# TheJacksonLaboratory/cnn_autoencoder

Measured on NVIDIA B200. Metric: wsi_encode_decode_megapixels_per_sec, higher is better.
Workload: dtype f16

## Files before the change

### cnn_autoencoder_b200/csrc/igemm_conv.cu

```cuda
#include <stdlib.h>
#include <string.h>

#include "cae_common.cuh"
#include "eb_device.cuh"

namespace {

constexpr int kMaxTaps = 9;
constexpr int kMaxSA = 6;
constexpr int kMaxSB = 12;
constexpr int kMaxEpiWarps = 12;
constexpr int kThreads = 128 + 32 * kMaxEpiWarps;

enum { EPI_ACT = 0, EPI_LATENT = 1, EPI_IMAGE = 2, EPI_PROJ = 3 };

constexpr int kProjN = 32;
constexpr int kProjK = 128;
constexpr int kProjStageBytes = (kProjK / 8) * 256 * 16;
constexpr int kProjWBytes = (kProjK / 8) * kProjN * 16;
__host__ __device__ inline int proj_slot(int kh, int kw) {
  const int slot[3][3] = {{12, 24, 27}, {16, 0, 3}, {19, 6, 9}};
  return slot[kh][kw];
}

struct IgTap {
  uint32_t a_off;
  uint32_t acc;
};

constexpr int kMaxItems = 18;
constexpr int kMaxStages = 9;

struct IgItem {
  uint32_t a_off16, b_off16, d_off, first;
};

struct IgParams {
  int n_img, dom_h, dom_w;
  int tiles_x, tiles_per_img, n_tiles;
  int mt, n_taps, n_chunks, ck;
  int N, n_acc, n_buf, tmem_cols;
  int PH, PW, n_par, par_stride;
  int a_stage_bytes, a_box_bytes, b_stage_bytes, sa, sb;
  int tpb, b_tap_bytes;
  int n_pass;
  int pass_tap0[2];
  int n_stages[2];
  IgItem items[2][2][kMaxItems];
  int item_start[2][2][kMaxStages + 1];
  int epi_warps;
  int debug;
  int org_y, org_x;
  uint32_t lbo_a, sbo_a, lbo_b, sbo_b, idesc;
  IgTap taps[kMaxTaps];
  const uint8_t *wpack;
  size_t wpack_half_bytes;
  int resident;
  uint32_t b_chunk16;
  int up;
  int c_out, pre_act, post_act;
  const float *bias;
  ActView out, skip;
  float *aux;
  int out_h, out_w;
  uint32_t out_pitch, out_ps, out_is, skip_pitch, skip_ps, skip_is;
  int pair_store;
  int quant;
  int q_smem;
  int q_core_min, q_core_len;
  cae_eb_tables qt;
  float *q_yq;
  int32_t *q_sym, *q_hist, *q_status;
  double *q_rate;
  ActView q_pl;
  uint32_t q_pitch, q_ps, q_is;
  const uint8_t *proj_w;
  __half *proj_out;
  uint32_t idesc2;
};

struct TapDef {
  int par, dy, dx, acc, kh, kw;
};

int build_taps(int kind, bool merged, TapDef *t) {
  int n = 0;
  if (kind == CAE_CONV_S1) {
    for (int kh = 0; kh < 3; ++kh)
      for (int kw = 0; kw < 3; ++kw) t[n++] = {0, kh, kw, 0, kh, kw};
  } else if (kind == CAE_CONV_S2) {
    for (int kh = 0; kh < 3; ++kh)
      for (int kw = 0; kw < 3; ++kw)
        t[n++] = {((kh & 1) << 1) | ((kw + CAE_COL_PAD) & 1), kh >> 1,
                  ((kw + CAE_COL_PAD) >> 1) - 1, 0, kh, kw};
  } else if (kind == CAE_CONVT_S1) {
    for (int dy = 0; dy < 3; ++dy)
      for (int dx = 0; dx < 3; ++dx) t[n++] = {0, dy, dx, 0, 2 - dy, 2 - dx};
  } else if (merged) {
    for (int dy = 0; dy < 2; ++dy)
      for (int dx = 0; dx < 2; ++dx) t[n++] = {0, dy, dx, 0, -1, -1};
  } else {
    for (int py = 0; py < 2; ++py)
      for (int px = 0; px < 2; ++px)
        for (int dy = 0; dy <= py; ++dy)
          for (int dx = 0; dx <= px; ++dx)
            t[n++] = {0, dy, dx, py * 2 + px, py + 1 - 2 * dy, px + 1 - 2 * dx};
  }
  return n;
}

inline int round_up(int a, int b) { return (a + b - 1) / b * b; }

inline bool is_merged(int kind, int c_out) { return kind == CAE_CONVT_S2 && 4 * c_out <= 16; }

inline int mma_n(int kind, int c_out) {
  return is_merged(kind, c_out) ? 16 : round_up(c_out, 16);
}

inline bool use_pair(int kind, int c_out) {
  return !is_merged(kind, c_out) && mma_n(kind, c_out) == 128 && cae_knob(CAE_KNOB_IGEMM_PAIR_MMA);
}

inline int auto_ck(int kind, int c_in_p, bool merged = false, bool pair = false) {
  if (pair && c_in_p % 32 == 0) {
    if (const char *e = cae_knob(CAE_KNOB_IGEMM_CK_PAIR)) {
      const int v = atoi(e);
      if ((v == 16 || v == 32 || v == 64) && c_in_p % v == 0) return v;
// ... 387 lines not shown
    return;
  }

#pragma unroll 1
  for (int part = 0; part < 2; ++part) {
    if (part == 1 && !second) break;
    float v[16];
#pragma unroll
    for (int i = 0; i < 16; ++i) v[i] = __uint_as_float(part ? r1[i] : r0[i]);
    const int c0 = part ? c_second : c_first;
    const int ox = ox0 + (p.up == 2 ? part : 0);
    if (p.bias) {
      if (c0 + 16 <= p.c_out) {
        const float4 *bp = reinterpret_cast<const float4 *>(p.bias + c0);
#pragma unroll
        for (int q = 0; q < 4; ++q) {
          const float4 bv = __ldg(bp + q);
          v[4 * q] += bv.x;
          v[4 * q + 1] += bv.y;
          v[4 * q + 2] += bv.z;
          v[4 * q + 3] += bv.w;
        }
      } else {
#pragma unroll
        for (int i = 0; i < 16; ++i)
          if (c0 + i < p.c_out) v[i] += __ldg(p.bias + c0 + i);
      }
    }
    if (pre_s != 1.f) {
#pragma unroll
      for (int i = 0; i < 16; ++i) v[i] = fmaxf(v[i], v[i] * pre_s);
    }
    if (p.skip.ptr) {
      const uint32_t off = pixel_unit(p.skip.fmt, p.skip_pitch, p.skip_ps, p.skip_is,
                                      p.skip.planes, n, oy + 1, ox + 1) +
                           (uint32_t)(c0 >> 3) * p.skip_ps;
      const uint4 *sp = reinterpret_cast<const uint4 *>(p.skip.ptr) + off;
#pragma unroll
      for (int h = 0; h < 2; ++h) {
        const uint4 sv = __ldg(sp + h * p.skip_ps);
        const __half2 *sh = reinterpret_cast<const __half2 *>(&sv);
#pragma unroll
        for (int k = 0; k < 4; ++k) {
          const float2 f = __half22float2(sh[k]);
          v[h * 8 + 2 * k] += f.x;
          v[h * 8 + 2 * k + 1] += f.y;
        }
      }
    }
    if (post_s != 1.f) {
#pragma unroll
      for (int i = 0; i < 16; ++i) v[i] = fmaxf(v[i], v[i] * post_s);
    }
    if (EPI == EPI_LATENT) {
      if (valid) {
        float *o = reinterpret_cast<float *>(p.out.ptr) +
                   (((size_t)n * p.c_out + c0) * p.out_h + oy) * p.out_w + ox;
        const size_t cs = (size_t)p.out_h * p.out_w;
#pragma unroll
        for (int i = 0; i < 16; ++i)
          if (c0 + i < p.c_out) o[i * cs] = v[i];
      }
      if (fused_q) quant_emit16(p, qs, v, c0, n, oy, ox, valid, q_bits);
    } else {
      const uint4 lo = pack8(v), hi = pack8(v + 8);
      const uint32_t off = pixel_unit(p.out.fmt, p.out_pitch, p.out_ps, p.out_is, p.out.planes,
                                      n, oy + 1, ox + 1) + (uint32_t)(c0 >> 3) * p.out_ps;
      uint4 *dst = reinterpret_cast<uint4 *>(p.out.ptr) + off;
      dst[0] = lo;
      dst[p.out_ps] = hi;
      if (p.out.halo == CAE_HALO_REFLECT &&
          (oy == 1 || oy == p.out.H - 2 || ox == 1 || ox == p.out.W - 2))
        store_halo2(p, n, c0 >> 3, oy, ox, lo, hi);
    }
  }
}

template <int EPI, int FAST, int PAIR>
__global__ void __launch_bounds__(EPI == EPI_PROJ ? 128 + 32 * 17 : (FAST == 1 ? 128 + 32 * 16 : kThreads), 1)
igemm_conv_kernel(const __grid_constant__ CUtensorMap tmA, const __grid_constant__ IgParams p) {
  extern __shared__ uint8_t smem_raw[];
  __shared__ __align__(8) uint64_t a_full[kMaxSA], a_empty[kMaxSA];
  __shared__ __align__(8) uint64_t b_full[kMaxSB], b_empty[kMaxSB];
  __shared__ __align__(8) uint64_t acc_full[2], acc_empty[2];
  __shared__ __align__(8) uint64_t b_peer[kMaxSB];
  __shared__ __align__(8) uint64_t u_full, u_free, d2_full;
  __shared__ uint32_t tmem_base_s;

  const int warp = threadIdx.x >> 5, lane = threadIdx.x & 31;
  const uint32_t rank = PAIR ? cluster_ctarank() : 0u;
  const int unit0 = PAIR ? (int)(blockIdx.x >> 1) : (int)blockIdx.x;
  const int unit_step = PAIR ? (int)(gridDim.x >> 1) : (int)gridDim.x;
  const int n_units = (PAIR ? (p.n_tiles + 1) >> 1 : p.n_tiles) * p.n_pass;
  const uint32_t smem_base = (smem_u32(smem_raw) + 1023u) & ~1023u;
  uint8_t *smem = smem_raw + (smem_base - smem_u32(smem_raw));
  uint8_t *smem_a = smem;
  uint8_t *smem_b = smem + (size_t)p.sa * p.a_stage_bytes;
  QuantSmem qs{nullptr, nullptr, nullptr};
  if (EPI == EPI_LATENT && p.quant && p.q_smem) {
    float *q0 = reinterpret_cast<float *>(smem_b + (size_t)p.sb * p.b_stage_bytes);
    const int nl = p.c_out * p.q_core_len, nh = p.q_hist ? nl : 0;
    for (int i = threadIdx.x; i < p.c_out; i += blockDim.x) q0[i] = p.qt.medians[i];
    for (int i = threadIdx.x; i < nl; i += blockDim.x) {
      const int c = i / p.q_core_len, k = i - c * p.q_core_len;
      q0[p.c_out + i] = p.qt.lut[(size_t)c * p.qt.lut_len + (p.q_core_min - p.qt.lut_min) + k];
    }
    int *h0 = reinterpret_cast<int *>(q0 + p.c_out + nl);
    for (int i = threadIdx.x; i < nh; i += blockDim.x) h0[i] = 0;
    qs.med = q0;
    qs.lut = q0 + p.c_out;
    qs.hist = nh ? h0 : nullptr;
  }

  if (threadIdx.x == 0) {
    for (int i = 0; i < p.sa; ++i) {
      mbar_init(&a_full[i], 1);
      mbar_init(&a_empty[i], 2);
    }
    for (int i = 0; i < p.sb; ++i) {
      mbar_init(&b_full[i], 1);
      mbar_init(&b_empty[i], 2);
    }
    for (int i = 0; i < 2; ++i) {
      mbar_init(&acc_full[i], 2);
      mbar_init(&acc_empty[i], (uint32_t)p.epi_warps * (PAIR ? 2u : 1u));
    }
    if (PAIR) {
      for (int i = 0; i < p.sb; ++i) mbar_init(&b_peer[i], 1);
    }
    if (EPI == EPI_PROJ) {
      mbar_init(&u_full, (uint32_t)p.epi_warps * (PAIR ? 2u : 1u));
      mbar_init(&u_free, 1);
      mbar_init(&d2_full, 1);
    }
    fence_barrier_init();
  }
  uint8_t *u_stage = smem_b + (size_t)p.sb * p.b_stage_bytes;
  uint8_t *proj_w_s = u_stage + kProjStageBytes;
  if (EPI == EPI_PROJ) {
    const uint4 *src = reinterpret_cast<const uint4 *>(
        p.proj_w + (PAIR ? kProjWBytes + rank * (kProjWBytes / 2) : 0));
    uint4 *dst = reinterpret_cast<uint4 *>(proj_w_s);
    for (int i = threadIdx.x; i < kProjWBytes / 16 / (PAIR ? 2 : 1); i += blockDim.x)
      dst[i] = __ldg(src + i);
    fence_proxy_async();
  }
  if (warp == 3) tmem_alloc_g<PAIR>(&tmem_base_s, (uint32_t)p.tmem_cols);
  if (warp == 0 && lane == 0) prefetch_tensormap(&tmA);
  tc_fence_before();
  if (PAIR) cluster_sync_all(); else __syncthreads();
  tc_fence_after();
  const uint32_t tmem_base = tmem_base_s;

  if (warp == 0) {
    if (lane == 0) {
      uint32_t it = 0;
      for (int vt = unit0; vt < n_units; vt += unit_step) {
        const int tile = PAIR ? (vt / p.n_pass) * 2 + (int)rank : vt / p.n_pass;
        const int n = tile / p.tiles_per_img, rem = tile - n * p.tiles_per_img;
        const int ty = rem / p.tiles_x, tx = rem - ty * p.tiles_x;
        const int y0 = ty * 16 + p.org_y, x0 = tx * 8 * p.mt + p.org_x;
        for (int ch = 0; ch < p.n_chunks; ++ch, ++it) {
          const int s = it % p.sa;
          mbar_wait(&a_empty[s], ((it / p.sa) & 1) ^ 1);
          if (PAIR) {
            if (rank == 0) mbar_expect_tx(&a_full[s], 2u * (uint32_t)(p.n_par * p.a_box_bytes));
            const uint32_t bar = mapa_u32(smem_u32(&a_full[s]), 0);
            for (int par = 0; par < p.n_par; ++par)
              tma_load_4d_pair(&tmA, bar,
                               smem_a + (size_t)s * p.a_stage_bytes + (size_t)par * p.par_stride,
                               x0 * 8, y0, ch * (p.ck >> 3), n * p.n_par + par);
            continue;
          }
          if (p.debug & 1) { mbar_arrive(&a_full[s]); continue; }
          mbar_expect_tx(&a_full[s], (uint32_t)(p.n_par * p.a_box_bytes));
          for (int par = 0; par < p.n_par; ++par)
            tma_load_4d(&tmA, &a_full[s],
                        smem_a + (size_t)s * p.a_stage_bytes + (size_t)par * p.par_stride, x0 * 8,
                        y0, ch * (p.ck >> 3), n * p.n_par + par);
        }
      }
    }
  } else if (warp == 1) {
    if (lane == 0) {
      uint32_t it = 0;
      const uint8_t *wsrc = p.wpack + (size_t)rank * p.wpack_half_bytes;
      if (p.resident) {
        mbar_expect_tx(&b_full[0], (uint32_t)p.b_stage_bytes);
        for (int k = 0; k < p.n_chunks * p.n_taps; ++k)
          bulk_load_1d(smem_b + (size_t)k * p.b_tap_bytes, wsrc + (size_t)k * p.b_tap_bytes,
                       (uint32_t)p.b_tap_bytes, &b_full[0]);
      }
      for (int vt = unit0; vt < n_units && !p.resident; vt += unit_step) {
        const int pass = vt % p.n_pass;
        for (int ch = 0; ch < p.n_chunks; ++ch) {
          for (int st = 0; st < p.n_stages[pass]; ++st, ++it) {
            const int s = it % p.sb;
            mbar_wait(&b_empty[s], ((it / p.sb) & 1) ^ 1);
            if (p.debug & 2) { mbar_arrive(&b_full[s]); continue; }
            mbar_expect_tx(&b_full[s], (uint32_t)p.b_stage_bytes);
            bulk_load_1d(smem_b + (size_t)s * p.b_stage_bytes,
                         wsrc + (size_t)(ch * p.n_taps + p.pass_tap0[pass] + st * p.tpb) *
                                    p.b_tap_bytes,
                         (uint32_t)p.b_stage_bytes, &b_full[s]);
          }
        }
      }
    }
  }
  if (PAIR && rank != 0 && (warp == 2 || warp == 3)) {
    if (warp == 3 && lane == 0) {
      if (p.resident) {
        mbar_wait(&b_full[0], 0);
        mbar_arrive_cluster(mapa_u32(smem_u32(&b_peer[0]), 0));
      }
      uint32_t it = 0;
      for (int vt = unit0; vt < n_units && !p.resident; vt += unit_step) {
        const int pass = vt % p.n_pass;
        for (int k = 0; k < p.n_chunks * p.n_stages[pass]; ++k, ++it) {
          const int s = it % p.sb;
          mbar_wait(&b_full[s], (it / p.sb) & 1);
          mbar_arrive_cluster(mapa_u32(smem_u32(&b_peer[s]), 0));
        }
      }
    }
  } else if (warp == 2 || warp == 3) {
    const int issuer = warp - 2;
    const bool leader = elect_one();
    const uint32_t a_hi = ((p.sbo_a >> 4) & 0x3FFFu) | (1u << 14);
    const uint32_t b_hi = ((p.sbo_b >> 4) & 0x3FFFu) | (1u << 14);
    const uint32_t a_lbo = ((p.lbo_a >> 4) & 0x3FFFu) << 16;
    const uint32_t b_lbo = ((p.lbo_b >> 4) & 0x3FFFu) << 16;
    const uint32_t a_kstep = (2 * p.lbo_a) >> 4, b_kstep = (2 * p.lbo_b) >> 4;
    const uint32_t sa_base = smem_base >> 4;
    const uint32_t sb_base = (smem_base + (uint32_t)(p.sa * p.a_stage_bytes)) >> 4;
    const uint32_t a_stage16 = (uint32_t)p.a_stage_bytes >> 4;
    const uint32_t b_stage16 = (uint32_t)p.b_stage_bytes >> 4;
    const uint32_t idesc = p.idesc;
    const int ksteps = p.ck >> 4;
    const uint32_t buf_cols = (uint32_t)(p.mt * p.n_acc * p.N);
    const bool no_mma = (p.debug & 4) != 0;
    uint32_t j = 0;
    int sA = 0, sB = 0;
    uint32_t phA = 0, phB = 0;
    const bool resident = p.resident != 0;
    if (resident) {
      mbar_wait(&b_full[0], 0);
      if (PAIR) mbar_wait_cluster(&b_peer[0], 0);
    }
    for (int vt = unit0; vt < n_units; vt += unit_step, ++j) {
      const int pass = vt % p.n_pass;
      const int n_stages = p.n_stages[pass];
      const int buf = j % p.n_buf;
      if (PAIR) mbar_wait_cluster(&acc_empty[buf], ((j / p.n_buf) & 1) ^ 1);
      else mbar_wait(&acc_empty[buf], ((j / p.n_buf) & 1) ^ 1);
      tc_fence_after();
      const uint32_t d_buf = tmem_base + (uint32_t)buf * buf_cols;
      for (int ch = 0; ch < p.n_chunks; ++ch) {
        if (PAIR) mbar_wait_cluster(&a_full[sA], phA); else mbar_wait(&a_full[sA], phA);
        const uint32_t a_stage = ((sa_base + (uint32_t)sA * a_stage16) & 0x3FFFu) | a_lbo;
        const uint32_t later = ch > 0 ? 1u : 0u;
        for (int st = 0; st < n_stages; ++st) {
          if (!resident) {
            mbar_wait(&b_full[sB], phB);
            if (PAIR) mbar_wait_cluster(&b_peer[sB], phB);
          }
          tc_fence_after();
          const uint32_t b_stage =
              ((sb_base + (resident ? (uint32_t)ch * p.b_chunk16 : (uint32_t)sB * b_stage16)) & 0x3FFFu) | b_lbo;
          const int i1 = p.item_start[pass][issuer][st + 1];
          for (int i = p.item_start[pass][issuer][st]; i < i1; ++i) {
            const IgItem it = p.items[pass][issuer][i];
            const uint32_t d = d_buf + it.d_off;
            uint32_t a_lo = a_stage + it.a_off16, b_lo = b_stage + it.b_off16;
            uint32_t flag = later | (it.first ^ 1u);
            if (leader && !no_mma) {
#pragma unroll 4
              for (int k = 0; k < ksteps; ++k) {
                umma_f16_lohi_g<PAIR>(d, a_lo, a_hi, b_lo, b_hi, idesc, flag);
                a_lo += a_kstep;
                b_lo += b_kstep;
                flag = 1u;
              }
            }
          }
          if (leader) {
            if (!resident) umma_commit_g<PAIR>(&b_empty[sB]);
            if (st == n_stages - 1) umma_commit_g<PAIR>(&a_empty[sA]);
            if (st == n_stages - 1 && ch == p.n_chunks - 1) umma_commit_g<PAIR>(&acc_full[buf]);
          }
          if (!resident && ++sB == p.sb) { sB = 0; phB ^= 1u; }
        }
        if (++sA == p.sa) { sA = 0; phA ^= 1u; }
      }
    }
  } else if (warp >= 4 && warp < 4 + p.epi_warps) {
    const int quad = warp & 3, half = (warp - 4) >> 2, n_halves = p.epi_warps >> 2;
    const int row = quad * 32 + lane;
    const int ty = row >> 3, txl = row & 7;
    const int acc_per_buf = p.mt * p.n_acc;
    const uint32_t lane_base = tmem_base + ((uint32_t)(quad * 32) << 16);
    int jobs_per_m;
    if (EPI == EPI_IMAGE) jobs_per_m = 1;
    else if (p.up == 1) jobs_per_m = (p.N + 31) >> 5;
    else jobs_per_m = (p.n_pass == 2 ? 1 : 2) * (p.N >> 4);
    const int n_jobs = p.mt * jobs_per_m;
    const float pre_s = act_slope(p.pre_act), post_s = act_slope(p.post_act);
    float q_bits = 0.f;
    uint32_t j = 0;
    const uint32_t u_full_addr = PAIR ? mapa_u32(smem_u32(&u_full), 0) : smem_u32(&u_full);
    const uint32_t acc_empty_addr0 = PAIR ? mapa_u32(smem_u32(&acc_empty[0]), 0) : 0u;
    const uint32_t acc_empty_addr1 = PAIR ? mapa_u32(smem_u32(&acc_empty[1]), 0) : 0u;
    for (int vt = unit0; vt < n_units; vt += unit_step, ++j) {
      const int pass = vt % p.n_pass;
      const int tile = PAIR ? (vt / p.n_pass) * 2 + (int)rank : vt / p.n_pass;
      const int n = tile / p.tiles_per_img, rem = tile - n * p.tiles_per_img;
      const int tyi = rem / p.tiles_x, txi = rem - tyi * p.tiles_x;
      const int buf = j % p.n_buf;
      const int y = tile < p.n_tiles ? tyi * 16 + ty : p.dom_h;
      if (FAST == 2 && p.up == 1 && (txl == 0 || txl == 7) && y < p.dom_h && !(p.debug & 64)) {
        for (int job = half; job < n_jobs; job += n_halves) {
          const int m = job / jobs_per_m, jj = job - m * jobs_per_m;
          const int x = (txi * p.mt + m) * 8 + txl;
          if (x >= p.dom_w) continue;
          const uint4 *sp = reinterpret_cast<const uint4 *>(p.skip.ptr) +
                            pixel_unit(p.skip.fmt, p.skip_pitch, p.skip_ps, p.skip_is,
                                       p.skip.planes, n, y + 1, x + 1) +
                            (uint32_t)(jj * 4) * p.skip_ps;
#pragma unroll
          for (int q = 0; q < 4; ++q)
            asm volatile("prefetch.global.L2 [%0];" ::"l"(sp + q * p.skip_ps));
        }
      }
      mbar_wait(&acc_full[buf], (j / p.n_buf) & 1);
      tc_fence_after();
      if (EPI == EPI_PROJ) {
        mbar_wait(&u_free, (j & 1u) ^ 1u);
        const __half2 pre2 = __float2half2_rn(pre_s), post2 = __float2half2_rn(post_s);
        for (int job = half; job < (kProjK >> 4); job += n_halves) {
          const int c_first = job * 16;
          uint32_t r0[16], r1[16];
          const uint32_t t = lane_base + (uint32_t)(buf * acc_per_buf * p.N + c_first);
          __syncwarp();
          tmem_ld16(t, r0);
          tmem_ld16(t + (uint32_t)p.N, r1);
          tmem_ld_wait();
          __half2 ha[8], hb[8];
          fast_half16<false>(p, r0, c_first, pre_s, pre2, post2, nullptr, ha);
          fast_half16<false>(p, r1, c_first, pre_s, pre2, post2, nullptr, hb);
          uint4 *dst = reinterpret_cast<uint4 *>(u_stage + (size_t)(c_first >> 3) * 4096) + row;
          dst[0] = make_uint4(h2u(ha[0]), h2u(ha[1]), h2u(ha[2]), h2u(ha[3]));
          dst[128] = make_uint4(h2u(hb[0]), h2u(hb[1]), h2u(hb[2]), h2u(hb[3]));
          dst[256] = make_uint4(h2u(ha[4]), h2u(ha[5]), h2u(ha[6]), h2u(ha[7]));
          dst[384] = make_uint4(h2u(hb[4]), h2u(hb[5]), h2u(hb[6]), h2u(hb[7]));
        }
        fence_proxy_async();
        tc_fence_before();
        __syncwarp();
        if (lane == 0) {
          if (PAIR) mbar_arrive_cluster(u_full_addr); else mbar_arrive(&u_full);
        }
        mbar_wait(&d2_full, j & 1u);
        tc_fence_after();
        const uint32_t d2 = lane_base + (uint32_t)(buf * acc_per_buf * p.N);
        const int x = txi * 8 + txl;
        for (int unit = half; unit < 4; unit += n_halves) {
          const int blk = unit >> 1, hh = unit & 1;
          uint32_t r[16];
          __syncwarp();
          tmem_ld16(d2 + (uint32_t)(blk * kProjN + hh * 16), r);
          tmem_ld_wait();
          if (y < p.dom_h && x < p.dom_w && !(p.debug & 8)) {
            __half *o = p.proj_out +
                        (((size_t)n * p.out_h + (y * 2 + pass)) * p.out_w + (x * 2 + blk)) * kProjN +
                        hh * 16;
            asm volatile("st.global.v8.b32 [%0], {%1,%2,%3,%4,%5,%6,%7,%8};" ::"l"(o),
                         "r"(pack2(__uint_as_float(r[0]), __uint_as_float(r[1]))),
                         "r"(pack2(__uint_as_float(r[2]), __uint_as_float(r[3]))),
                         "r"(pack2(__uint_as_float(r[4]), __uint_as_float(r[5]))),
                         "r"(pack2(__uint_as_float(r[6]), __uint_as_float(r[7]))),
                         "r"(pack2(__uint_as_float(r[8]), __uint_as_float(r[9]))),
                         "r"(pack2(__uint_as_float(r[10]), __uint_as_float(r[11]))),
                         "r"(pack2(__uint_as_float(r[12]), __uint_as_float(r[13]))),
                         "r"(pack2(__uint_as_float(r[14]), __uint_as_float(r[15])))
                         : "memory");
          }
        }
        tc_fence_before();
        __syncwarp();
        if (lane == 0) {
        if (PAIR) mbar_arrive_cluster_relaxed(buf ? acc_empty_addr1 : acc_empty_addr0); else mbar_arrive(&acc_empty[buf]);
      }
        continue;
      }
      for (int job = half; job < n_jobs; job += n_halves) {
        const int m = job / jobs_per_m, jj = job - m * jobs_per_m;
        const int x = (txi * p.mt + m) * 8 + txl;
        const bool valid = y < p.dom_h && x < p.dom_w;
        epilogue_job<EPI, FAST>(p, lane_base, buf * acc_per_buf + m * p.n_acc, n, y, x, jj, valid,
                                pre_s, post_s, pass, qs, q_bits);
      }
      tc_fence_before();
      __syncwarp();
      if (lane == 0) {
        if (PAIR) mbar_arrive_cluster_relaxed(buf ? acc_empty_addr1 : acc_empty_addr0); else mbar_arrive(&acc_empty[buf]);
      }
    }
    if (EPI == EPI_LATENT && p.quant && p.q_rate) {
      for (int o = 16; o > 0; o >>= 1) q_bits += __shfl_xor_sync(0xffffffffu, q_bits, o);
      if (lane == 0 && q_bits != 0.f) atomicAdd(p.q_rate, (double)q_bits);
    }
  } else if (EPI == EPI_PROJ && warp == 4 + p.epi_warps && rank == 0) {
    const bool leader = elect_one();
    const uint32_t us = smem_u32(u_stage), ws = smem_u32(proj_w_s);
    const uint32_t buf_cols = (uint32_t)(p.mt * p.n_acc * p.N);
    uint32_t j = 0;
    constexpr uint32_t kRowsB = kProjN / (PAIR ? 2 : 1);
    for (int vt = unit0; vt < n_units; vt += unit_step, ++j) {
      if (PAIR) mbar_wait_cluster(&u_full, j & 1u); else mbar_wait(&u_full, j & 1u);
      tc_fence_after();
      if (leader) {
        const uint32_t d2 = tmem_base + (j % (uint32_t)p.n_buf) * buf_cols;
#pragma unroll
        for (int blk = 0; blk < 2; ++blk) {
#pragma unroll
          for (int k = 0; k < kProjK / 16; ++k) {
            const uint64_t da = make_smem_desc(us + blk * 2048 + k * 8192, 4096, 128);
            const uint64_t db = make_smem_desc(ws + k * (2 * kRowsB * 16), kRowsB * 16, 128);
            umma_f16_g<PAIR>(d2 + blk * kProjN, da, db, p.idesc2, k > 0 ? 1u : 0u);
          }
        }
        umma_commit_g<PAIR>(&u_free);
        umma_commit_g<PAIR>(&d2_full);
      }
      __syncwarp();
    }
  }

  tc_fence_before();
  if (PAIR) cluster_sync_all(); else __syncthreads();
  if (EPI == EPI_LATENT && qs.hist) {
    const int nh = p.c_out * p.q_core_len, bins = p.qt.hist_bins;
    for (int i = threadIdx.x; i < nh; i += blockDim.x) {
      const int v = qs.hist[i];
      if (v) {
        const int c = i / p.q_core_len;
        int b = p.q_core_min + (i - c * p.q_core_len) - p.qt.hist_min;
        b = b < 0 ? 0 : (b >= bins ? bins - 1 : b);
        atomicAdd(p.q_hist + (size_t)c * bins + b, v);
      }
    }
  }
  if (warp == 3) tmem_dealloc_g<PAIR>(tmem_base, (uint32_t)p.tmem_cols);
}

__global__ void pack_proj_kernel(const float *__restrict__ w, const float *__restrict__ scale,
                                 int c_out, __half *__restrict__ out) {
  const int i = blockIdx.x * blockDim.x + threadIdx.x;
  if (i >= kProjK * kProjN) return;
  const int k8 = i & 7, n = (i >> 3) % kProjN, kplane = i / (8 * kProjN);
  const int ci = kplane * 8 + k8;
  float v = 0.f;
  for (int kh = 0; kh < 3; ++kh)
    for (int kw = 0; kw < 3; ++kw) {
      const int c = n - proj_slot(kh, kw);
      if (c >= 0 && c < c_out && c < 3)
        v = w[(((size_t)ci * c_out + c) * 3 + kh) * 3 + kw] * (scale ? scale[c] : 1.f);
    }
  out[i] = __float2half_rn(v);
  const int half = kProjN / 2, r = n / half;
  out[kProjK * kProjN + r * (kProjK * half) + (kplane * half + (n - r * half)) * 8 + k8] =
      __float2half_rn(v);
}

struct ProjGatherParams {
  const uint4 *proj;
  int n, h, w, c_out;
  const float *bias;
  float pre_s, post_s;
  uint8_t *out;
  float *aux;
};

__device__ __forceinline__ void unpack8(const uint4 &u, float (&f)[8]) {
  const __half2 *h = reinterpret_cast<const __half2 *>(&u);
#pragma unroll
  for (int k = 0; k < 4; ++k) {
    const float2 t = __half22float2(h[k]);
// ... 75 lines not shown

EncodeTiledFn get_encode_fn() {
  static EncodeTiledFn fn = nullptr;
  if (!fn) {
    void *ptr = nullptr;
    cudaDriverEntryPointQueryResult qres;
    if (cudaGetDriverEntryPoint("cuTensorMapEncodeTiled", &ptr, cudaEnableDefault, &qres) ==
            cudaSuccess &&
        qres == cudaDriverEntryPointSuccess)
      fn = reinterpret_cast<EncodeTiledFn>(ptr);
  }
  return fn;
}

int pow2_cols(int c) {
  int r = 32;
  while (r < c) r <<= 1;
  return r;
}

}

extern "C" size_t cae_packed_weight_bytes(int kind, int c_in, int c_out, int ck) {
  const int c_in_p = round_up(c_in, 16);
  if (ck <= 0) ck = auto_ck(kind, c_in_p, is_merged(kind, c_out), use_pair(kind, c_out));
  TapDef taps[kMaxTaps];
  const int n_taps = build_taps(kind, is_merged(kind, c_out), taps);
  return (size_t)(c_in_p / ck) * n_taps * mma_n(kind, c_out) * ck * sizeof(__half);
}

extern "C" int cae_pack_weights(int kind, int c_in, int c_out, int ck, const float *w,
                                const float *scale, void *packed, void *stream) {
  CAE_CHECK(kind >= CAE_CONV_S1 && kind <= CAE_CONVT_S2, 2, "cae_pack_weights: bad kind %d", kind);
  CAE_CHECK(w && packed, 2, "cae_pack_weights: null pointer");
  const int c_in_p = round_up(c_in, 16);
  if (ck <= 0) ck = auto_ck(kind, c_in_p, is_merged(kind, c_out), use_pair(kind, c_out));
  CAE_CHECK(ck % 16 == 0 && ck <= 128 && c_in_p % ck == 0, 2,
            "cae_pack_weights: ck=%d does not divide padded c_in=%d", ck, c_in_p);
  PackParams q;
  memset(&q, 0, sizeof(q));
  q.kind = kind;
  q.merged = is_merged(kind, c_out);
  q.c_in = c_in;
  q.c_out = c_out;
  q.ck = ck;
  q.N = mma_n(kind, c_out);
  q.n_taps = build_taps(kind, q.merged, q.taps);
  q.n_chunks = c_in_p / ck;
  q.pair = use_pair(kind, c_out) ? 1 : 0;
  const size_t total = (size_t)q.n_chunks * q.n_taps * q.N * ck;
  const int threads = 256;
  pack_weights_kernel<<<(unsigned)((total + threads - 1) / threads), threads, 0,
                        (cudaStream_t)stream>>>(q, w, scale, (__half *)packed, total);
  cae_count_launch();
  CAE_CUDA(cudaGetLastError());
  return 0;
}

extern "C" int cae_conv_igemm(const cae_conv_desc *d, void *stream) {
  CAE_CHECK(d, 2, "cae_conv_igemm: null descriptor");
  const int kind = d->kind;
  CAE_CHECK(kind >= CAE_CONV_S1 && kind <= CAE_CONVT_S2, 2, "cae_conv_igemm: bad kind %d", kind);
  CAE_CHECK(d->in.ptr && d->weights, 2, "cae_conv_igemm: null input or weights");
  CAE_CHECK(d->groups <= 1, 2, "cae_conv_igemm: grouped convolutions run on cae_conv_direct");
  CAE_CHECK(d->n > 0 && d->h_in > 0 && d->w_in > 0, 2, "cae_conv_igemm: bad shape");
  const int c_in_p = round_up(d->c_in, 16);
  CAE_CHECK(d->in.planes * 8 == c_in_p, 2,
            "cae_conv_igemm: input has %d planes, need %d (c_in padded to 16)", d->in.planes,
            c_in_p / 8);
  const bool merged = is_merged(kind, d->c_out);
  const int want_fmt = kind == CAE_CONV_S2 ? CAE_FMT_F16_SPLIT : CAE_FMT_F16_PLANAR;
  CAE_CHECK(d->in.fmt == want_fmt, 2, "cae_conv_igemm: input format %d, kind %d needs %d",
            d->in.fmt, kind, want_fmt);
  if (kind == CAE_CONV_S2)
    CAE_CHECK(d->h_in % 2 == 0 && d->w_in % 2 == 0, 2,
              "cae_conv_igemm: stride-2 conv needs even input size, got %dx%d", d->h_in, d->w_in);

  IgParams p;
  memset(&p, 0, sizeof(p));
  p.n_img = d->n;
  p.N = mma_n(kind, d->c_out);
  CAE_CHECK(p.N <= 256, 2, "cae_conv_igemm: c_out=%d too large", d->c_out);
  const bool pair = use_pair(kind, d->c_out);
  p.ck = d->ck > 0 ? d->ck : auto_ck(kind, c_in_p, merged, pair);
  CAE_CHECK(p.ck % 16 == 0 && p.ck <= 128 && c_in_p % p.ck == 0, 2, "cae_conv_igemm: bad ck=%d",
            p.ck);
  p.n_chunks = c_in_p / p.ck;
  CAE_CHECK(!(pair && d->out.fmt == CAE_FMT_F32_NCHW), 2,
            "cae_conv_igemm: a 128-channel fp32 latent layer is not covered by the CTA-pair form "
            "(unset CAE_IGEMM_PAIR_MMA)");
  TapDef taps[kMaxTaps];
  p.n_taps = build_taps(kind, merged, taps);
  const bool convt2 = kind == CAE_CONVT_S2 && !merged;
  p.n_pass = 1;
  if (convt2 && (cae_knob(CAE_KNOB_IGEMM_TWO_PASS) || (4 * p.N > 256 && !cae_knob(CAE_KNOB_IGEMM_ONE_PASS))))
    p.n_pass = 2;
  p.n_acc = (kind == CAE_CONVT_S2 && !merged) ? (p.n_pass == 2 ? 2 : 4) : 1;
  p.up = (kind == CAE_CONVT_S2) ? 2 : 1;

  if (kind == CAE_CONV_S2) {
    p.dom_h = d->h_in / 2;
    p.dom_w = d->w_in / 2;
  } else {
    p.dom_h = d->h_in;
    p.dom_w = d->w_in;
  }
  p.out_h = p.dom_h * p.up;
  p.out_w = p.dom_w * p.up;

  int mt = d->mt > 0 ? d->mt : 2;
  if (d->mt <= 0)
    if (const char *e = cae_knob(CAE_KNOB_IGEMM_MT)) mt = atoi(e) == 1 ? 1 : 2;
  if (p.dom_w <= 8) mt = 1;
  if (p.n_acc * p.N * mt > 512) mt = 1;
  if (p.n_pass == 2 && p.n_acc * p.N * mt > 256) mt = 1;
  CAE_CHECK(p.n_acc * p.N * mt <= 512, 2, "cae_conv_igemm: accumulators exceed TMEM");
  p.mt = mt;
  p.n_buf = (512 / (p.n_acc * p.N * mt)) >= 2 ? 2 : 1;
  p.tmem_cols = pow2_cols(p.n_buf * p.n_acc * p.N * mt);

  if (kind == CAE_CONV_S1 || kind == CAE_CONVT_S1) {
    p.PH = 18;
    p.PW = 8 * mt + 2;
    p.n_par = 1;
    p.org_y = 0;
    p.org_x = CAE_COL_PAD;
  } else if (kind == CAE_CONV_S2) {
    p.PH = 17;
    p.PW = 8 * mt + 1;
    p.n_par = 4;
    p.org_y = 0;
    p.org_x = 1;
  } else {
    p.PH = 17;
    p.PW = 8 * mt + 1;
    p.n_par = 1;
    p.org_y = 1;
    p.org_x = 1 + CAE_COL_PAD;
  }
  const int kplanes = p.ck / 8;
  p.a_box_bytes = kplanes * p.PH * p.PW * 16;
  p.par_stride = round_up(p.a_box_bytes, 128);
  p.a_stage_bytes = round_up(p.par_stride * p.n_par, 128);
  p.lbo_a = (uint32_t)(p.PH * p.PW * 16);
  p.sbo_a = (uint32_t)(p.PW * 16);
  p.lbo_b = (uint32_t)((pair ? p.N / 2 : p.N) * 16);
  p.sbo_b = 128;
  if (cae_knob(CAE_KNOB_IGEMM_SWAP_LBO_SBO)) {
    uint32_t t = p.lbo_a; p.lbo_a = p.sbo_a; p.sbo_a = t;
    t = p.lbo_b; p.lbo_b = p.sbo_b; p.sbo_b = t;
  }
  p.idesc = make_idesc_f16(pair ? 256 : 128, p.N);
  for (int t = 0; t < p.n_taps; ++t) {
    p.taps[t].a_off = (uint32_t)(taps[t].par * p.par_stride + (taps[t].dy * p.PW + taps[t].dx) * 16);
    p.taps[t].acc = (uint32_t)taps[t].acc;
  }

  int budget = 227 * 1024 - 2048;
  int q_bytes = 0;
  if (d->quant && d->out.fmt == CAE_FMT_F32_NCHW && !merged && d->quant->tables.lut &&
      !cae_knob(CAE_KNOB_QUANT_NO_SMEM)) {
    const cae_eb_tables &t = d->quant->tables;
    int core = (40 * 1024 / (4 * d->c_out) - 1) / 2;
    if (core > t.lut_len) core = t.lut_len;
    if (core >= 16) {
      int cmin = -(core / 2);
      if (cmin < t.lut_min) cmin = t.lut_min;
      if (cmin + core > t.lut_min + t.lut_len) cmin = t.lut_min + t.lut_len - core;
      p.q_core_min = cmin;
      p.q_core_len = core;
      q_bytes = round_up(4 * d->c_out * (1 + 2 * core), 128);
    }
  }
  budget -= q_bytes;
  const bool proj = d->proj != nullptr;
  if (proj) {
    CAE_CHECK(convt2 && p.n_pass == 2 && p.mt == 1 && p.N == kProjK && d->c_out == kProjK, 2,
              "cae_conv_igemm(proj): needs ConvTranspose2d stride 2 with %d output channels", kProjK);
    CAE_CHECK(d->proj->weights && d->proj->proj, 2, "cae_conv_igemm(proj): null pointer");
    CAE_CHECK(!d->skip.ptr && !d->quant && !d->aux_out, 2,
              "cae_conv_igemm(proj): no skip / quantizer / aux output on a projected layer");
    budget -= kProjStageBytes + kProjWBytes;
  }
  p.b_tap_bytes = (pair ? p.N / 2 : p.N) * p.ck * 2;
  p.wpack_half_bytes = (size_t)p.n_chunks * p.n_taps * p.b_tap_bytes;
  int pass_ntaps[2] = {p.n_taps, 0};
  p.pass_tap0[0] = p.pass_tap0[1] = 0;
  if (p.n_pass == 2) {
    pass_ntaps[0] = 0;
    for (int t = 0; t < p.n_taps; ++t) pass_ntaps[taps[t].acc >> 1]++;
    p.pass_tap0[1] = pass_ntaps[0];
  }
  auto divides = [&](int v) {
    return pass_ntaps[0] % v == 0 && (p.n_pass == 1 || pass_ntaps[1] % v == 0);
  };
  const int resident_bytes = p.n_chunks * p.n_taps * p.b_tap_bytes;
  const bool resident = pair && !cae_knob(CAE_KNOB_IGEMM_NO_RESIDENT) &&
                        resident_bytes + 2 * p.a_stage_bytes <= budget;
  p.resident = resident ? 1 : 0;
  p.b_chunk16 = (uint32_t)((p.n_taps * p.b_tap_bytes) >> 4);
  int tpb = 1;
  for (int cand = p.n_taps; cand >= 1 && !resident; --cand) {
    if (!divides(cand)) continue;
    if (2 * p.a_stage_bytes + 2 * cand * p.b_tap_bytes <= budget && cand * p.b_tap_bytes <= 73728) {
      tpb = cand;
      break;
    }
  }
  if (const char *e = resident ? nullptr : cae_knob(CAE_KNOB_IGEMM_TPB)) {
    const int v = atoi(e);
    if (v >= 1 && divides(v) && 2 * p.a_stage_bytes + 2 * v * p.b_tap_bytes <= budget) tpb = v;
  }
  p.tpb = tpb;
  p.b_stage_bytes = resident ? resident_bytes : tpb * p.b_tap_bytes;
  for (int ps = 0; ps < p.n_pass; ++ps) {
    if (resident) tpb = pass_ntaps[ps];
    const int b_tap0 = resident ? p.pass_tap0[ps] : 0;
    p.n_stages[ps] = pass_ntaps[ps] / tpb;
    CAE_CHECK(p.n_stages[ps] <= kMaxStages, 2, "cae_conv_igemm: too many weight stages");
    int cnt[2] = {0, 0};
    uint32_t seen = 0;
    for (int st = 0; st < p.n_stages[ps]; ++st) {
      p.item_start[ps][0][st] = cnt[0];
      p.item_start[ps][1][st] = cnt[1];
      for (int tt = 0; tt < tpb; ++tt) {
        const int t = p.pass_tap0[ps] + st * tpb + tt;
        for (int m = 0; m < p.mt; ++m) {
          const int acc = m * p.n_acc + (p.n_pass == 2 ? (taps[t].acc & 1) : taps[t].acc);
          const int who = acc & 1;
          CAE_CHECK(cnt[who] < kMaxItems, 2, "cae_conv_igemm: work list overflow");
          IgItem &it = p.items[ps][who][cnt[who]++];
          it.a_off16 = (uint32_t)((taps[t].par * p.par_stride + (taps[t].dy * p.PW + taps[t].dx) * 16 +
                                   m * 128) >> 4);
          it.b_off16 = (uint32_t)(((b_tap0 + tt) * p.b_tap_bytes) >> 4);
          it.d_off = (uint32_t)(acc * p.N);
          it.first = (seen >> acc) & 1u ? 0u : 1u;
          seen |= 1u << acc;
        }
      }
    }
    p.item_start[ps][0][p.n_stages[ps]] = cnt[0];
    p.item_start[ps][1][p.n_stages[ps]] = cnt[1];
  }
  int sa = 2, sb = resident ? 1 : 2;
  CAE_CHECK(sa * p.a_stage_bytes + sb * p.b_stage_bytes <= budget, 2,
            "cae_conv_igemm: tile does not fit shared memory (A %d B %d)", p.a_stage_bytes,
            p.b_stage_bytes);
  for (;;) {
    bool grew = false;
    const int sb_max = resident ? 1 : kMaxSB;
    if (sb < 3 && sb < sb_max && sa * p.a_stage_bytes + (sb + 1) * p.b_stage_bytes <= budget) { ++sb; grew = true; }
    else if (sa < 3 && (sa + 1) * p.a_stage_bytes + sb * p.b_stage_bytes <= budget) { ++sa; grew = true; }
    else if (sb < 4 && sb < sb_max && sa * p.a_stage_bytes + (sb + 1) * p.b_stage_bytes <= budget) { ++sb; grew = true; }
    else if (sa < 4 && (sa + 1) * p.a_stage_bytes + sb * p.b_stage_bytes <= budget) { ++sa; grew = true; }
    else if (sa < kMaxSA && (sa + 1) * p.a_stage_bytes + sb * p.b_stage_bytes <= budget) { ++sa; grew = true; }
    else if (sb < sb_max && sa * p.a_stage_bytes + (sb + 1) * p.b_stage_bytes <= budget) { ++sb; grew = true; }
    if (!grew) break;
  }
  p.sa = sa;
  p.sb = sb;
  const int smem_bytes = sa * p.a_stage_bytes + sb * p.b_stage_bytes + 1024 + q_bytes +
                         (proj ? kProjStageBytes + kProjWBytes : 0);
  p.q_smem = q_bytes > 0;
  p.tiles_x = (p.dom_w + 8 * mt - 1) / (8 * mt);
  const int tiles_y = (p.dom_h + 15) / 16;
  p.tiles_per_img = p.tiles_x * tiles_y;
  p.n_tiles = p.tiles_per_img * d->n;
  if (cae_knob(CAE_KNOB_IGEMM_VERBOSE))
    fprintf(stderr, "cae_conv_igemm: kind %d %d->%d @%dx%d N=%d ck=%d mt=%d n_pass=%d n_acc=%d n_buf=%d "
            "tpb=%d a_stage=%d x%d b_stage=%d x%d smem=%d tiles=%d pair=%d resident=%d\n", kind, d->c_in, d->c_out, d->h_in,
            d->w_in, p.N, p.ck, p.mt, p.n_pass, p.n_acc, p.n_buf, p.tpb, p.a_stage_bytes, sa,
            p.b_stage_bytes, sb, smem_bytes, p.n_tiles, (int)pair, p.resident);

  p.wpack = (const uint8_t *)d->weights;

  p.c_out = d->c_out;
  p.pre_act = d->pre_act;
  p.post_act = d->post_act;
  p.bias = d->bias;
  p.aux = (float *)d->aux_out;
  int epi;
  if (proj) {
    epi = EPI_PROJ;
    p.proj_w = (const uint8_t *)d->proj->weights;
    p.proj_out = (__half *)d->proj->proj;
    p.idesc2 = make_idesc_f16(pair ? 256 : 128, kProjN);
  } else if (merged) {
    epi = EPI_IMAGE;
    CAE_CHECK(d->out.fmt == CAE_FMT_U8_HWC || d->out.fmt == CAE_FMT_NONE, 2,
              "cae_conv_igemm: final layer writes U8_HWC (and/or aux fp32)");
    CAE_CHECK(d->out.ptr || d->aux_out, 2, "cae_conv_igemm: no output");
    p.out.ptr = d->out.fmt == CAE_FMT_U8_HWC ? d->out.ptr : nullptr;
  } else if (d->out.fmt == CAE_FMT_F32_NCHW) {
    epi = EPI_LATENT;
    CAE_CHECK(p.up == 1 && d->out.ptr, 2, "cae_conv_igemm: fp32 NCHW output needs up==1");
    p.out.ptr = d->out.ptr;
    if (d->quant) {
      const cae_quant_fuse *q = d->quant;
      CAE_CHECK(!d->skip.ptr, 2, "cae_conv_igemm: fused quantizer on a residual layer");
      if (int rc = eb_check_tables(&q->tables, "cae_conv_igemm(quant)")) return rc;
      CAE_CHECK(q->tables.hist_bins >= 0 && q->tables.hist_bins <= 8192, 2,
                "cae_conv_igemm(quant): hist_bins out of range");
      p.quant = 1;
      p.qt = q->tables;
      p.q_yq = q->y_q;
      p.q_sym = q->symbols;
      p.q_hist = q->hist;
      p.q_rate = q->rate_bits;
      p.q_status = q->status;
      if (cae_knob(CAE_KNOB_QUANT_NO_HIST)) p.q_hist = nullptr;
      if (cae_knob(CAE_KNOB_QUANT_NO_RATE)) p.q_rate = nullptr;
      if (cae_knob(CAE_KNOB_QUANT_NO_YQ)) p.q_yq = nullptr;
      if (q->y_q_planar.fmt != CAE_FMT_NONE && q->y_q_planar.ptr) {
        CAE_CHECK(q->y_q_planar.fmt == CAE_FMT_F16_PLANAR && q->y_q_planar.planes * 8 == p.N, 2,
                  "cae_conv_igemm(quant): planar y_q needs %d planes", p.N / 8);
        p.q_pl = ActView{q->y_q_planar.ptr, q->y_q_planar.fmt, q->y_q_planar.planes,
                         q->y_q_planar.halo, p.out_h, p.out_w};
      }
    }
  } else {
    epi = EPI_ACT;
    CAE_CHECK(d->out.ptr && (d->out.fmt == CAE_FMT_F16_PLANAR || d->out.fmt == CAE_FMT_F16_SPLIT),
              2, "cae_conv_igemm: bad output format %d", d->out.fmt);
    CAE_CHECK(d->out.planes * 8 == p.N, 2, "cae_conv_igemm: output has %d planes, need %d",
              d->out.planes, p.N / 8);
    if (d->out.fmt == CAE_FMT_F16_SPLIT)
      CAE_CHECK(p.out_h % 2 == 0 && p.out_w % 2 == 0, 2, "cae_conv_igemm: split output needs even size");
    p.out.ptr = d->out.ptr;
  }
  p.out.fmt = proj ? CAE_FMT_NONE : d->out.fmt;
  p.out.planes = d->out.planes;
  p.out.halo = d->out.halo;
  p.out.H = p.out_h;
  p.out.W = p.out_w;
  auto strides = [](int fmt, int planes, int H, int W, uint32_t &pitch, uint32_t &ps,
                    uint32_t &is) {
    if (fmt == CAE_FMT_F16_SPLIT) {
      pitch = (uint32_t)(cae_row_units(W) / 2);
      ps = pitch * (uint32_t)((H + 2) / 2);
      is = 4u * (uint32_t)planes * ps;
    } else {
      pitch = (uint32_t)cae_row_units(W);
      ps = pitch * (uint32_t)(H + 2);
      is = (uint32_t)planes * ps;
    }
  };
  if (epi == EPI_ACT) {
    CAE_CHECK(!d->aux_out, 2, "cae_conv_igemm: aux_out is only available on the final image layer");
    CAE_CHECK((double)d->n * d->out.planes * (p.out_h + 2) * cae_row_units(p.out_w) < 2147483648.0, 2,
              "cae_conv_igemm: output tensor too large for 32-bit unit offsets; split the batch");
    strides(p.out.fmt, p.out.planes, p.out_h, p.out_w, p.out_pitch, p.out_ps, p.out_is);
  }
  if (p.q_pl.ptr) strides(p.q_pl.fmt, p.q_pl.planes, p.out_h, p.out_w, p.q_pitch, p.q_ps, p.q_is);
  if (d->skip.fmt != CAE_FMT_NONE && d->skip.ptr) {
    CAE_CHECK(epi != EPI_IMAGE, 2, "cae_conv_igemm: skip unsupported on the final layer");
// ... 133 lines not shown
```

Measured before the change: 4952.

## Add mt=4 staggered tile mode with per-slot accumulator barriers for stride-2 convs

For stride-2 convolutions with N=128, the tile width grows to four 8-pixel M-subtiles. The A loads are split into two TMA x-boxes, and the channel chunk shrinks to 16, with the packed weights sub-indexed per tap. Each accumulator slot gets its own full/empty mbarrier, so the epilogue can drain one subtile while the MMA is still writing the others. The aim is to overlap epilogue and MMA and to reuse weights across a wider tile. The cost is more barriers, smaller K chunks and more TMA issues per stage.

```diff
diff --git a/cnn_autoencoder_b200/csrc/igemm_conv.cu b/cnn_autoencoder_b200/csrc/igemm_conv.cu
--- a/cnn_autoencoder_b200/csrc/igemm_conv.cu
+++ b/cnn_autoencoder_b200/csrc/igemm_conv.cu
@@ -30,9 +30,10 @@
 
 constexpr int kMaxItems = 18;
 constexpr int kMaxStages = 9;
+constexpr int kMaxSlots = 8;
 
 struct IgItem {
-  uint32_t a_off16, b_off16, d_off, first;
+  uint32_t a_off16, b_off16, d_off, flags;
 };
 
 struct IgParams {
@@ -43,6 +44,9 @@
   int PH, PW, n_par, par_stride;
   int a_stage_bytes, a_box_bytes, b_stage_bytes, sa, sb;
   int tpb, b_tap_bytes;
+  int b_sub;
+  int n_xbox;
+  int stagger;
   int n_pass;
   int pass_tap0[2];
   int n_stages[2];
@@ -596,13 +600,14 @@
   extern __shared__ uint8_t smem_raw[];
   __shared__ __align__(8) uint64_t a_full[kMaxSA], a_empty[kMaxSA];
   __shared__ __align__(8) uint64_t b_full[kMaxSB], b_empty[kMaxSB];
-  __shared__ __align__(8) uint64_t acc_full[2], acc_empty[2];
+  __shared__ __align__(8) uint64_t acc_full[kMaxSlots], acc_empty[kMaxSlots];
   __shared__ __align__(8) uint64_t b_peer[kMaxSB];
   __shared__ __align__(8) uint64_t u_full, u_free, d2_full;
   __shared__ uint32_t tmem_base_s;
 
   const int warp = threadIdx.x >> 5, lane = threadIdx.x & 31;
   const uint32_t rank = PAIR ? cluster_ctarank() : 0u;
+  const bool stagger = EPI != EPI_PROJ && !PAIR && p.stagger;
   const int unit0 = PAIR ? (int)(blockIdx.x >> 1) : (int)blockIdx.x;
   const int unit_step = PAIR ? (int)(gridDim.x >> 1) : (int)gridDim.x;
   const int n_units = (PAIR ? (p.n_tiles + 1) >> 1 : p.n_tiles) * p.n_pass;
@@ -635,8 +640,8 @@
       mbar_init(&b_full[i], 1);
       mbar_init(&b_empty[i], 2);
     }
-    for (int i = 0; i < 2; ++i) {
-      mbar_init(&acc_full[i], 2);
+    for (int i = 0; i < kMaxSlots; ++i) {
+      mbar_init(&acc_full[i], stagger ? 1 : 2);
       mbar_init(&acc_empty[i], (uint32_t)p.epi_warps * (PAIR ? 2u : 1u));
     }
     if (PAIR) {
@@ -687,11 +692,14 @@
             continue;
           }
           if (p.debug & 1) { mbar_arrive(&a_full[s]); continue; }
-          mbar_expect_tx(&a_full[s], (uint32_t)(p.n_par * p.a_box_bytes));
+          mbar_expect_tx(&a_full[s], (uint32_t)(p.n_par * p.n_xbox * p.a_box_bytes));
+          const int xb_step = 8 * p.mt / p.n_xbox;
           for (int par = 0; par < p.n_par; ++par)
-            tma_load_4d(&tmA, &a_full[s],
-                        smem_a + (size_t)s * p.a_stage_bytes + (size_t)par * p.par_stride, x0 * 8,
-                        y0, ch * (p.ck >> 3), n * p.n_par + par);
+            for (int xb = 0; xb < p.n_xbox; ++xb)
+              tma_load_4d(&tmA, &a_full[s],
+                          smem_a + (size_t)s * p.a_stage_bytes +
+                              (size_t)(par * p.n_xbox + xb) * p.par_stride,
+                          (x0 + xb * xb_step) * 8, y0, ch * (p.ck >> 3), n * p.n_par + par);
         }
       }
     }
@@ -713,10 +721,19 @@
             mbar_wait(&b_empty[s], ((it / p.sb) & 1) ^ 1);
             if (p.debug & 2) { mbar_arrive(&b_full[s]); continue; }
             mbar_expect_tx(&b_full[s], (uint32_t)p.b_stage_bytes);
-            bulk_load_1d(smem_b + (size_t)s * p.b_stage_bytes,
-                         wsrc + (size_t)(ch * p.n_taps + p.pass_tap0[pass] + st * p.tpb) *
-                                    p.b_tap_bytes,
-                         (uint32_t)p.b_stage_bytes, &b_full[s]);
+            const int pc = ch / p.b_sub, sub = ch - pc * p.b_sub;
+            const uint8_t *src =
+                wsrc + ((size_t)(pc * p.n_taps + p.pass_tap0[pass] + st * p.tpb) * p.b_sub + sub) *
+                           p.b_tap_bytes;
+            if (p.b_sub == 1) {
+              bulk_load_1d(smem_b + (size_t)s * p.b_stage_bytes, src, (uint32_t)p.b_stage_bytes,
+                           &b_full[s]);
+            } else {
+              for (int tt = 0; tt < p.tpb; ++tt)
+                bulk_load_1d(smem_b + (size_t)s * p.b_stage_bytes + (size_t)tt * p.b_tap_bytes,
+                             src + (size_t)tt * p.b_sub * p.b_tap_bytes, (uint32_t)p.b_tap_bytes,
+                             &b_full[s]);
+            }
           }
         }
       }
@@ -766,9 +783,12 @@
       const int pass = vt % p.n_pass;
       const int n_stages = p.n_stages[pass];
       const int buf = j % p.n_buf;
-      if (PAIR) mbar_wait_cluster(&acc_empty[buf], ((j / p.n_buf) & 1) ^ 1);
-      else mbar_wait(&acc_empty[buf], ((j / p.n_buf) & 1) ^ 1);
-      tc_fence_after();
+      const uint32_t empty_par = ((j / p.n_buf) & 1) ^ 1;
+      if (!stagger) {
+        if (PAIR) mbar_wait_cluster(&acc_empty[buf], empty_par);
+        else mbar_wait(&acc_empty[buf], empty_par);
+        tc_fence_after();
+      }
       const uint32_t d_buf = tmem_base + (uint32_t)buf * buf_cols;
       for (int ch = 0; ch < p.n_chunks; ++ch) {
         if (PAIR) mbar_wait_cluster(&a_full[sA], phA); else mbar_wait(&a_full[sA], phA);
@@ -785,9 +805,14 @@
           const int i1 = p.item_start[pass][issuer][st + 1];
           for (int i = p.item_start[pass][issuer][st]; i < i1; ++i) {
             const IgItem it = p.items[pass][issuer][i];
+            const uint32_t slot = (uint32_t)buf * (uint32_t)p.mt + (it.flags >> 2);
+            if (stagger && ch == 0 && (it.flags & 1u)) {
+              mbar_wait(&acc_empty[slot], empty_par);
+              tc_fence_after();
+            }
             const uint32_t d = d_buf + it.d_off;
             uint32_t a_lo = a_stage + it.a_off16, b_lo = b_stage + it.b_off16;
-            uint32_t flag = later | (it.first ^ 1u);
+            uint32_t flag = later | ((it.flags & 1u) ^ 1u);
             if (leader && !no_mma) {
 #pragma unroll 4
               for (int k = 0; k < ksteps; ++k) {
@@ -797,11 +822,14 @@
                 flag = 1u;
               }
             }
+            if (leader && stagger && ch == p.n_chunks - 1 && (it.flags & 2u))
+              umma_commit_g<PAIR>(&acc_full[slot]);
           }
           if (leader) {
             if (!resident) umma_commit_g<PAIR>(&b_empty[sB]);
             if (st == n_stages - 1) umma_commit_g<PAIR>(&a_empty[sA]);
-            if (st == n_stages - 1 && ch == p.n_chunks - 1) umma_commit_g<PAIR>(&acc_full[buf]);
+            if (!stagger && st == n_stages - 1 && ch == p.n_chunks - 1)
+              umma_commit_g<PAIR>(&acc_full[buf]);
           }
           if (!resident && ++sB == p.sb) { sB = 0; phB ^= 1u; }
         }
@@ -846,9 +874,10 @@
             asm volatile("prefetch.global.L2 [%0];" ::"l"(sp + q * p.skip_ps));
         }
       }
-      mbar_wait(&acc_full[buf], (j / p.n_buf) & 1);
-      tc_fence_after();
+      const uint32_t full_par = (j / p.n_buf) & 1;
       if (EPI == EPI_PROJ) {
+        mbar_wait(&acc_full[buf], full_par);
+        tc_fence_after();
         mbar_wait(&u_free, (j & 1u) ^ 1u);
         const __half2 pre2 = __float2half2_rn(pre_s), post2 = __float2half2_rn(post_s);
         for (int job = half; job < (kProjK >> 4); job += n_halves) {
@@ -907,17 +936,23 @@
       }
         continue;
       }
-      for (int job = half; job < n_jobs; job += n_halves) {
-        const int m = job / jobs_per_m, jj = job - m * jobs_per_m;
-        const int x = (txi * p.mt + m) * 8 + txl;
-        const bool valid = y < p.dom_h && x < p.dom_w;
-        epilogue_job<EPI, FAST>(p, lane_base, buf * acc_per_buf + m * p.n_acc, n, y, x, jj, valid,
-                                pre_s, post_s, pass, qs, q_bits);
-      }
-      tc_fence_before();
-      __syncwarp();
-      if (lane == 0) {
-        if (PAIR) mbar_arrive_cluster_relaxed(buf ? acc_empty_addr1 : acc_empty_addr0); else mbar_arrive(&acc_empty[buf]);
+      const int n_grp = stagger ? p.mt : 1, grp_jobs = n_jobs / n_grp;
+      for (int g = 0; g < n_grp; ++g) {
+        const int slot = stagger ? buf * p.mt + g : buf;
+        mbar_wait(&acc_full[slot], full_par);
+        tc_fence_after();
+        for (int job = g * grp_jobs + half; job < (g + 1) * grp_jobs; job += n_halves) {
+          const int m = job / jobs_per_m, jj = job - m * jobs_per_m;
+          const int x = (txi * p.mt + m) * 8 + txl;
+          const bool valid = y < p.dom_h && x < p.dom_w;
+          epilogue_job<EPI, FAST>(p, lane_base, buf * acc_per_buf + m * p.n_acc, n, y, x, jj, valid,
+                                  pre_s, post_s, pass, qs, q_bits);
+        }
+        tc_fence_before();
+        __syncwarp();
+        if (lane == 0) {
+          if (PAIR) mbar_arrive_cluster_relaxed(buf ? acc_empty_addr1 : acc_empty_addr0); else mbar_arrive(&acc_empty[slot]);
+        }
       }
     }
     if (EPI == EPI_LATENT && p.quant && p.q_rate) {
@@ -1159,10 +1194,9 @@
   p.N = mma_n(kind, d->c_out);
   CAE_CHECK(p.N <= 256, 2, "cae_conv_igemm: c_out=%d too large", d->c_out);
   const bool pair = use_pair(kind, d->c_out);
-  p.ck = d->ck > 0 ? d->ck : auto_ck(kind, c_in_p, merged, pair);
-  CAE_CHECK(p.ck % 16 == 0 && p.ck <= 128 && c_in_p % p.ck == 0, 2, "cae_conv_igemm: bad ck=%d",
-            p.ck);
-  p.n_chunks = c_in_p / p.ck;
+  const int pack_ck = d->ck > 0 ? d->ck : auto_ck(kind, c_in_p, merged, pair);
+  CAE_CHECK(pack_ck % 16 == 0 && pack_ck <= 128 && c_in_p % pack_ck == 0, 2,
+            "cae_conv_igemm: bad ck=%d", pack_ck);
   CAE_CHECK(!(pair && d->out.fmt == CAE_FMT_F32_NCHW), 2,
             "cae_conv_igemm: a 128-channel fp32 latent layer is not covered by the CTA-pair form "
             "(unset CAE_IGEMM_PAIR_MMA)");
@@ -1188,29 +1222,40 @@
   int mt = d->mt > 0 ? d->mt : 2;
   if (d->mt <= 0)
     if (const char *e = cae_knob(CAE_KNOB_IGEMM_MT)) mt = atoi(e) == 1 ? 1 : 2;
-  if (p.dom_w <= 8) mt = 1;
-  if (p.n_acc * p.N * mt > 512) mt = 1;
+  if (d->mt <= 0 && !cae_knob(CAE_KNOB_IGEMM_MT) && kind == CAE_CONV_S2 && p.N == 128 && !pair &&
+      (d->ck <= 0 || d->ck == 16) && p.dom_w > 16 && round_up(p.dom_w, 32) == round_up(p.dom_w, 16))
+    mt = 4;
+  if (mt != 1 && mt != 4) mt = 2;
+  if (mt == 4 && (p.n_acc != 1 || pair)) mt = 2;
+  if (p.dom_w <= 8 && mt == 2) mt = 1;
+  while (mt > 1 && p.n_acc * p.N * mt > 512) mt = mt == 4 ? 2 : 1;
   if (p.n_pass == 2 && p.n_acc * p.N * mt > 256) mt = 1;
   CAE_CHECK(p.n_acc * p.N * mt <= 512, 2, "cae_conv_igemm: accumulators exceed TMEM");
   p.mt = mt;
   p.n_buf = (512 / (p.n_acc * p.N * mt)) >= 2 ? 2 : 1;
   p.tmem_cols = pow2_cols(p.n_buf * p.n_acc * p.N * mt);
+  p.stagger = mt == 4 ? 1 : 0;
+  p.n_xbox = mt == 4 ? 2 : 1;
+  p.ck = (mt == 4 && d->ck <= 0) ? 16 : pack_ck;
+  p.b_sub = pack_ck / p.ck;
+  p.n_chunks = c_in_p / p.ck;
+  const int bm = mt / p.n_xbox;
 
   if (kind == CAE_CONV_S1 || kind == CAE_CONVT_S1) {
     p.PH = 18;
-    p.PW = 8 * mt + 2;
+    p.PW = 8 * bm + 2;
     p.n_par = 1;
     p.org_y = 0;
     p.org_x = CAE_COL_PAD;
   } else if (kind == CAE_CONV_S2) {
     p.PH = 17;
-    p.PW = 8 * mt + 1;
+    p.PW = 8 * bm + 1;
     p.n_par = 4;
     p.org_y = 0;
     p.org_x = 1;
   } else {
     p.PH = 17;
-    p.PW = 8 * mt + 1;
+    p.PW = 8 * bm + 1;
     p.n_par = 1;
     p.org_y = 1;
     p.org_x = 1 + CAE_COL_PAD;
@@ -1218,7 +1263,7 @@
   const int kplanes = p.ck / 8;
   p.a_box_bytes = kplanes * p.PH * p.PW * 16;
   p.par_stride = round_up(p.a_box_bytes, 128);
-  p.a_stage_bytes = round_up(p.par_stride * p.n_par, 128);
+  p.a_stage_bytes = round_up(p.par_stride * p.n_par * p.n_xbox, 128);
   p.lbo_a = (uint32_t)(p.PH * p.PW * 16);
   p.sbo_a = (uint32_t)(p.PW * 16);
   p.lbo_b = (uint32_t)((pair ? p.N / 2 : p.N) * 16);
@@ -1297,25 +1342,29 @@
     CAE_CHECK(p.n_stages[ps] <= kMaxStages, 2, "cae_conv_igemm: too many weight stages");
     int cnt[2] = {0, 0};
     uint32_t seen = 0;
+    IgItem *last[kMaxSlots] = {};
     for (int st = 0; st < p.n_stages[ps]; ++st) {
       p.item_start[ps][0][st] = cnt[0];
       p.item_start[ps][1][st] = cnt[1];
-      for (int tt = 0; tt < tpb; ++tt) {
+      for (int k = 0; k < tpb * p.mt; ++k) {
+        const int tt = p.stagger ? k % tpb : k / p.mt, m = p.stagger ? k / tpb : k % p.mt;
         const int t = p.pass_tap0[ps] + st * tpb + tt;
-        for (int m = 0; m < p.mt; ++m) {
-          const int acc = m * p.n_acc + (p.n_pass == 2 ? (taps[t].acc & 1) : taps[t].acc);
-          const int who = acc & 1;
-          CAE_CHECK(cnt[who] < kMaxItems, 2, "cae_conv_igemm: work list overflow");
-          IgItem &it = p.items[ps][who][cnt[who]++];
-          it.a_off16 = (uint32_t)((taps[t].par * p.par_stride + (taps[t].dy * p.PW + taps[t].dx) * 16 +
-                                   m * 128) >> 4);
-          it.b_off16 = (uint32_t)(((b_tap0 + tt) * p.b_tap_bytes) >> 4);
-          it.d_off = (uint32_t)(acc * p.N);
-          it.first = (seen >> acc) & 1u ? 0u : 1u;
-          seen |= 1u << acc;
-        }
-      }
-    }
+        const int acc = m * p.n_acc + (p.n_pass == 2 ? (taps[t].acc & 1) : taps[t].acc);
+        const int who = acc & 1;
+        CAE_CHECK(cnt[who] < kMaxItems && acc < kMaxSlots, 2, "cae_conv_igemm: work list overflow");
+        IgItem &it = p.items[ps][who][cnt[who]++];
+        const int box = m / bm;
+        it.a_off16 = (uint32_t)(((taps[t].par * p.n_xbox + box) * p.par_stride +
+                                 (taps[t].dy * p.PW + taps[t].dx) * 16 + (m - box * bm) * 128) >> 4);
+        it.b_off16 = (uint32_t)(((b_tap0 + tt) * p.b_tap_bytes) >> 4);
+        it.d_off = (uint32_t)(acc * p.N);
+        it.flags = ((seen >> acc) & 1u ? 0u : 1u) | ((uint32_t)acc << 2);
+        seen |= 1u << acc;
+        last[acc] = &it;
+      }
+    }
+    for (int a = 0; a < kMaxSlots; ++a)
+      if (last[a]) last[a]->flags |= 2u;
     p.item_start[ps][0][p.n_stages[ps]] = cnt[0];
     p.item_start[ps][1][p.n_stages[ps]] = cnt[1];
   }
@@ -1344,10 +1393,11 @@
   p.tiles_per_img = p.tiles_x * tiles_y;
   p.n_tiles = p.tiles_per_img * d->n;
   if (cae_knob(CAE_KNOB_IGEMM_VERBOSE))
-    fprintf(stderr, "cae_conv_igemm: kind %d %d->%d @%dx%d N=%d ck=%d mt=%d n_pass=%d n_acc=%d n_buf=%d "
-            "tpb=%d a_stage=%d x%d b_stage=%d x%d smem=%d tiles=%d pair=%d resident=%d\n", kind, d->c_in, d->c_out, d->h_in,
-            d->w_in, p.N, p.ck, p.mt, p.n_pass, p.n_acc, p.n_buf, p.tpb, p.a_stage_bytes, sa,
-            p.b_stage_bytes, sb, smem_bytes, p.n_tiles, (int)pair, p.resident);
+    fprintf(stderr, "cae_conv_igemm: kind %d %d->%d @%dx%d N=%d ck=%d (packed %d) mt=%d stagger=%d "
+            "n_pass=%d n_acc=%d n_buf=%d tpb=%d stages/chunk=%d a_stage=%d x%d b_stage=%d x%d smem=%d "
+            "tiles=%d pair=%d resident=%d\n", kind, d->c_in, d->c_out, d->h_in, d->w_in, p.N, p.ck,
+            pack_ck, p.mt, p.stagger, p.n_pass, p.n_acc, p.n_buf, p.tpb, p.n_stages[0],
+            p.a_stage_bytes, sa, p.b_stage_bytes, sb, smem_bytes, p.n_tiles, (int)pair, p.resident);
 
   p.wpack = (const uint8_t *)d->weights;
 
```

Measured after the change: 4498 (median of 6 runs). 9.2% lower.
